# hermanjakobsen/robotic-ultrasound-imaging

Measured on AMD Instinct MI355X. Metric: env-steps/sec (whole node) at 4096 envs/GPU, random-action rollout, higher is better.
Workload: dtype f32

## Files before the change

### robotic-ultrasound-imaging_amd/csrc/usim_contact.h

```cpp
#pragma once

#define EB(off) lds[TB_WORDS + eb * GE_STRIDE + (off)]

DI float row_ror8(float x) { return __int_as_float(__builtin_amdgcn_update_dpp(0, __float_as_int(x), 0x128, 0xf, 0xf, true)); }
template <int D> DI float row_shr(float x) { return __int_as_float(__builtin_amdgcn_update_dpp(0, __float_as_int(x), 0x110 + D, 0xf, 0xf, true)); }

template <int G>
DI float group_allsum(float x) {
    if constexpr (G == 16) x += row_ror8(x);
    x += __int_as_float(__builtin_amdgcn_update_dpp(0, __float_as_int(x), 0x141, 0xf, 0xf, true));
    x += __int_as_float(__builtin_amdgcn_update_dpp(0, __float_as_int(x), 0xB1, 0xf, 0xf, true));
    x += __int_as_float(__builtin_amdgcn_update_dpp(0, __float_as_int(x), 0x4E, 0xf, 0xf, true));
    return x;
}

typedef float v2f __attribute__((ext_vector_type(2)));
struct b2 { bool x, y; };
template <class T> struct LaneVec;
template <> struct LaneVec<float> {
    typedef bool mask;
    static DI float splat(float a) { return a; }
    static DI float fma(float a, float b, float c) { return fmaf(a, b, c); }
    static DI float rcp(float a) { return rcp_(a); }
    static DI float rsq(float a) { return rsq_(a); }
    static DI float max(float a, float b) { return fmaxf(a, b); }
    static DI float min(float a, float b) { return fminf(a, b); }
    static DI bool gt(float a, float b) { return a > b; }
    static DI bool lt(float a, float b) { return a < b; }
    static DI bool both(bool a, bool b) { return bool(int(a) & int(b)); }
    static DI float sel(bool c, float a, float b) { return c ? a : b; }
    static DI float hsum(float a) { return a; }
    static DI float nsum(float a) { return -a; }
};
template <> struct LaneVec<v2f> {
    typedef b2 mask;
    static DI v2f splat(float a) { return (v2f)(a); }
    static DI v2f fma(v2f a, v2f b, v2f c) { return __builtin_elementwise_fma(a, b, c); }
    static DI v2f rcp(v2f a) { v2f r; r.x = rcp_(a.x); r.y = rcp_(a.y); return r; }
    static DI v2f rsq(v2f a) { v2f r; r.x = rsq_(a.x); r.y = rsq_(a.y); return r; }
    static DI v2f max(v2f a, v2f b) { v2f r; r.x = fmaxf(a.x, b.x); r.y = fmaxf(a.y, b.y); return r; }
    static DI v2f min(v2f a, v2f b) { v2f r; r.x = fminf(a.x, b.x); r.y = fminf(a.y, b.y); return r; }
    static DI b2 gt(v2f a, v2f b) { return b2{a.x > b.x, a.y > b.y}; }
    static DI b2 lt(v2f a, v2f b) { return b2{a.x < b.x, a.y < b.y}; }
    static DI b2 both(b2 a, b2 b) { return b2{bool(int(a.x) & int(b.x)), bool(int(a.y) & int(b.y))}; }
    static DI v2f sel(b2 c, v2f a, v2f b) { v2f r; r.x = c.x ? a.x : b.x; r.y = c.y ? a.y : b.y; return r; }
    static DI float hsum(v2f a) { return a.x + a.y; }
    static DI float nsum(v2f a) { return -a.x - a.y; }
};

template <class T>
DI typename LaneVec<T>::mask cone_local(const T b00, const T b01, const T b02, const T b11, const T b12, const T b22, T r0, T r1, T r2,
                                        const T f0, const T f1, const T f2, const T mu, T& lam, T& h0, T& h1, T& h2) {
    typedef LaneVec<T> V;
    const T Bf0 = V::fma(b02, f2, V::fma(b01, f1, b00 * f0)), Bf1 = V::fma(b12, f2, V::fma(b11, f1, b01 * f0)), Bf2 = V::fma(b22, f2, V::fma(b12, f1, b02 * f0));
    const T vr = V::fma(f2, r2, V::fma(f1, r1, f0 * r0)), vBv = V::fma(f2, Bf2, V::fma(f1, Bf1, f0 * Bf0));
    const T x = V::sel(V::gt(f0, V::splat(1e-10f)), V::max(-vr * V::rcp(vBv), V::splat(-1.f)), V::splat(0.f));
    r0 = V::fma(x, Bf0, r0); r1 = V::fma(x, Bf1, r1); r2 = V::fma(x, Bf2, r2);
    T n0 = V::fma(x, f0, f0), n1 = V::fma(x, f1, f1), n2 = V::fma(x, f2, f2);
    const T rt2 = V::fma(r1, r1, r2 * r2);
    const T irt = V::rsq(V::max(rt2, V::splat(1e-30f))), rtn = rt2 * irt;
    const T sl = V::sel(V::both(V::gt(rt2, V::splat(0.f)), V::lt(r0, mu * rtn)), -mu * irt, V::splat(0.f));
    const T u1 = sl * r1, u2 = sl * r2;
    const T Bu0 = V::fma(b02, u2, V::fma(b01, u1, b00)), Bu1 = V::fma(b12, u2, V::fma(b11, u1, b01)), Bu2 = V::fma(b22, u2, V::fma(b12, u1, b02));
    const T ur = V::fma(u2, r2, V::fma(u1, r1, r0)), uBu = V::fma(u2, Bu2, V::fma(u1, Bu1, Bu0));
    const T x2 = V::max(-ur * V::rcp(uBu), V::splat(0.f));
    n0 += x2; n1 = V::fma(x2, u1, n1); n2 = V::fma(x2, u2, n2);
    r1 = V::fma(x2, Bu1, r1); r2 = V::fma(x2, Bu2, r2);
    const T lim = mu * n0;
    const typename V::mask haslim = V::gt(lim, V::splat(1e-7f));
    const T q1 = r1 - V::fma(b12, n2, b11 * n1), q2 = r2 - V::fma(b22, n2, b12 * n1);
    T m11 = b11 + lam, m22 = b22 + lam, det = V::fma(m11, m22, -(b12 * b12));
    T a1 = V::fma(m22, q1, -(b12 * q2)), a2 = V::fma(m11, q2, -(b12 * q1));
    {
        const T aa = V::fma(a1, a1, a2 * a2);
        const T aAa = V::fma(m11 * a2, a2, V::fma(m22 * a1, a1, -2.f * b12 * a1 * a2));
        const T an = aa * V::rsq(V::max(aa, V::splat(1e-30f)));
        lam = V::max(V::fma(V::fma(-det, lim, an) * aa, V::rcp(V::max(lim * aAa, V::splat(1e-30f))), lam), V::splat(0.f));
    }
    m11 = b11 + lam; m22 = b22 + lam; det = V::fma(m11, m22, -(b12 * b12));
    a1 = V::fma(m22, q1, -(b12 * q2)); a2 = V::fma(m11, q2, -(b12 * q1));
    const T aa = V::fma(a1, a1, a2 * a2);
    const T sc = -V::min(lim * V::rsq(aa), V::rcp(det));
    h0 = n0; h1 = V::sel(haslim, a1 * sc, V::splat(0.f)); h2 = V::sel(haslim, a2 * sc, V::splat(0.f));
    return haslim;
}

DI void contact_row_geometry(const float* lds, const int eb, const int cl, const bool own, const DevModel& M, const DevCfg& C, const int nc, const int* cel, const float vz,
                             float (&w)[3][6], float (&g)[3], float (&Rd)[3], float (&Km)[MAXC], float (&vrel0)[3], float& ae0, float& kdist) {
#pragma unroll
    for (int c = 0; c < MAXC; ++c) Km[c] = 0.f;
#pragma unroll
    for (int d = 0; d < 3; ++d) {
        g[d] = 0.f; Rd[d] = 0.f; vrel0[d] = 0.f;
#pragma unroll
        for (int a = 0; a < 6; ++a) w[d][a] = 0.f;
    }
    ae0 = 0.f; kdist = 0.f;
    if (own) {
        const int b = GE_CG + cl * CG_WORDS;
        f3 nn = mk(EB(b + 0), EB(b + 1), EB(b + 2)), rr = mk(EB(b + 3), EB(b + 4), EB(b + 5));
        const int e = __float_as_int(EB(b + 6));
        const float dist = EB(b + 7);
        const float aa = -rcp_(1.f + nn.z), bb = nn.x * nn.y * aa;
        f3 t1 = mk(1.f + nn.x * nn.x * aa, bb, -nn.x);
        f3 t2 = mk(bb, 1.f + nn.y * nn.y * aa, -nn.y);
        f3 ax = mk(lds[TB_AXIS + 3 * e], lds[TB_AXIS + 3 * e + 1], lds[TB_AXIS + 3 * e + 2]);
        const float sde = EB(GE_SD + e);
        float xx = fminf(-dist * (1.0f / SI_WIDTH), 1.f);
        float yy = (xx < 0.5f) ? 2.f * xx * xx : 1.f - 2.f * (1.f - xx) * (1.f - xx);
        float dimp = SI_D0 + yy * (SI_DMAX - SI_D0);
        float kk = dimp * (1.0f / (SI_DMAX * SI_DMAX * SR_TC * SR_TC));
        float Rn = (1.f - dimp) * rcp_(dimp) * M.invw;
#pragma unroll
        for (int c = 0; c < MAXC; ++c) { const float t = lds[TB_LINV + e * LROW + cel[c]] * (1.0f / ELEM_MASS); Km[c] = (c < nc) ? t : 0.f; }
        ae0 = EB(GE_A + e);
        kdist = kk * dist;
#pragma unroll
        for (int d = 0; d < 3; ++d) {
            f3 dir = (d == 0) ? nn : (d == 1 ? t1 : t2);
            f3 rx = cross(rr, dir);
            w[d][0] = dir.x; w[d][1] = dir.y; w[d][2] = dir.z; w[d][3] = rx.x; w[d][4] = rx.y; w[d][5] = rx.z;
            g[d] = -dot(dir, ax);
            vrel0[d] = g[d] * sde - dir.z * vz;
            Rd[d] = (d == 0) ? Rn * C.rn_scale : Rn * (1.0f / IMPRATIO);
        }
    }
}
DI void contact_row_residual(const bool own, const float* Li, const float* alpha, const float* vs, const float (&w)[3][6], const float (&g)[3], const float (&vrel0)[3],
                             const float ae0, const float kdist, float (&Liw)[3][6], float (&cres)[3]) {
#pragma unroll
    for (int d = 0; d < 3; ++d) {
        cres[d] = 0.f;
#pragma unroll
        for (int a = 0; a < 6; ++a) Liw[d][a] = 0.f;
    }
    if (own) {
        const float bcon = 2.0f / (SI_DMAX * SR_TC);
#pragma unroll
        for (int d = 0; d < 3; ++d) {
// ... 87 lines not shown
        pub[4] = make_float4(Liw[2][4], Liw[2][5], g[0], g[1]); pub[5] = make_float4(g[2], 0.f, 0.f, 0.f);
    }
    group_sync();
}
DI void load_record(const float* lds, const int eb, const int k, float4 (&rk)[6]) {
    const float4* src = reinterpret_cast<const float4*>(&EB(k * 24));
#pragma unroll
    for (int v = 0; v < 6; ++v) rk[v] = src[v];
}
DI void delassus_block(const float (&w)[3][6], const float (&g)[3], const float (&Lk)[3][6], const float (&gk)[3], float (&Bj)[3][3]) {
#pragma unroll
    for (int dd = 0; dd < 3; ++dd) {
#pragma unroll
        for (int d = 0; d < 3; ++d) {
            float r1 = fmaf(w[d][4], Lk[dd][4], fmaf(w[d][2], Lk[dd][2], w[d][0] * Lk[dd][0]));
            float r2 = fmaf(w[d][5], Lk[dd][5], fmaf(w[d][3], Lk[dd][3], w[d][1] * Lk[dd][1]));
            Bj[d][dd] = fmaf(g[d], gk[dd], r1 + r2);
        }
    }
}
struct Sym3 { float b00, b01, b02, b11, b12, b22; };
template <bool CLONE, int NB>
DI void delassus_blocks(const float* lds, const int eb, const int gl, const int cl, const int ncr, const float (&w)[3][6], const float (&g)[3], const float (&Rd)[3],
                        const float (&Km)[MAXC], float (&B)[NB][3][3], Sym3& bd) {
    const bool upper = CLONE && gl >= 8 && ncr > 4;
    const int k0 = upper ? 4 : 0;
    bd = Sym3{0.f, 0.f, 0.f, 0.f, 0.f, 0.f};
    float4 rk[6];
    load_record(lds, eb, k0, rk);
#pragma unroll
    for (int j = 0; j < NB; ++j) {
        if (j < ncr) {
            float Kmj = Km[j];
            if constexpr (CLONE) Kmj = upper ? Km[4 + j] : Km[j];
            const float Lk[3][6] = {{rk[0].x, rk[0].y, rk[0].z, rk[0].w, rk[1].x, rk[1].y}, {rk[1].z, rk[1].w, rk[2].x, rk[2].y, rk[2].z, rk[2].w},
                                    {rk[3].x, rk[3].y, rk[3].z, rk[3].w, rk[4].x, rk[4].y}};
            const float gk[3] = {rk[4].z * Kmj, rk[4].w * Kmj, rk[5].x * Kmj};
            if (j + 1 < NB) load_record(lds, eb, k0 + j + 1, rk);
            delassus_block(w, g, Lk, gk, B[j]);
            const bool me = (cl - k0) == j;
            bd.b00 = me ? B[j][0][0] : bd.b00; bd.b01 = me ? B[j][0][1] : bd.b01; bd.b02 = me ? B[j][0][2] : bd.b02;
            bd.b11 = me ? B[j][1][1] : bd.b11; bd.b12 = me ? B[j][1][2] : bd.b12; bd.b22 = me ? B[j][2][2] : bd.b22;
        }
    }
    if constexpr (CLONE) {
        if (ncr > 4) {
            bd.b00 += row_ror8(bd.b00); bd.b01 += row_ror8(bd.b01); bd.b02 += row_ror8(bd.b02);
            bd.b11 += row_ror8(bd.b11); bd.b12 += row_ror8(bd.b12); bd.b22 += row_ror8(bd.b22);
        }
    }
    bd.b00 += Rd[0]; bd.b11 += Rd[1]; bd.b22 += Rd[2];
}

template <int G, bool CLONE, int NCM, int NB>
DI void delassus_product(const float (&B)[NB][3][3], const float D0, const float D1, const float D2, float& q0, float& q1, float& q2) {
    q0 = 0.f; q1 = 0.f; q2 = 0.f;
    if constexpr (NCM <= 4) {
#pragma unroll
        for (int k = 0; k < NCM; ++k) {
            const float e0 = group_bcast<G>(D0, k), e1 = group_bcast<G>(D1, k), e2 = group_bcast<G>(D2, k);
            q0 = fmaf(B[k][0][2], e2, fmaf(B[k][0][1], e1, fmaf(B[k][0][0], e0, q0)));
            q1 = fmaf(B[k][1][2], e2, fmaf(B[k][1][1], e1, fmaf(B[k][1][0], e0, q1)));
            q2 = fmaf(B[k][2][2], e2, fmaf(B[k][2][1], e1, fmaf(B[k][2][0], e0, q2)));
        }
    } else if constexpr (CLONE) {
#pragma unroll
        for (int j = 0; j < 4; ++j) {
            const float e0 = half_bcast(D0, j), e1 = half_bcast(D1, j), e2 = half_bcast(D2, j);
            q0 = fmaf(B[j][0][2], e2, fmaf(B[j][0][1], e1, fmaf(B[j][0][0], e0, q0)));
            q1 = fmaf(B[j][1][2], e2, fmaf(B[j][1][1], e1, fmaf(B[j][1][0], e0, q1)));
            q2 = fmaf(B[j][2][2], e2, fmaf(B[j][2][1], e1, fmaf(B[j][2][0], e0, q2)));
        }
        q0 += row_ror8(q0); q1 += row_ror8(q1); q2 += row_ror8(q2);
    } else {
        float h0 = 0.f, h1 = 0.f, h2 = 0.f;
#pragma unroll
        for (int k = 0; k < NCM; ++k) {
            const float e0 = group_bcast<G>(D0, k), e1 = group_bcast<G>(D1, k), e2 = group_bcast<G>(D2, k);
            float& a0 = (k < 4) ? q0 : h0; float& a1 = (k < 4) ? q1 : h1; float& a2 = (k < 4) ? q2 : h2;
            a0 = fmaf(B[k][0][2], e2, fmaf(B[k][0][1], e1, fmaf(B[k][0][0], e0, a0)));
            a1 = fmaf(B[k][1][2], e2, fmaf(B[k][1][1], e1, fmaf(B[k][1][0], e0, a1)));
            a2 = fmaf(B[k][2][2], e2, fmaf(B[k][2][1], e1, fmaf(B[k][2][0], e0, a2)));
        }
        q0 += h0; q1 += h1; q2 += h2;
    }
}

template <bool CLONE> using ContactLane = typename std::conditional<CLONE, float, v2f>::type;

template <int G, bool CLONE, bool WARM, int NCM, int NB>
DI void jacobi_iterations(const int iters, const float (&B)[NB][3][3], const Sym3& bd, const float (&Rd)[3], const typename LaneVec<ContactLane<CLONE>>::mask ownv,
                          const ContactLane<CLONE> muv, ContactLane<CLONE> (&fv)[3], ContactLane<CLONE>& lamv, float (&cres)[3]) {
    typedef ContactLane<CLONE> VT;
    typedef LaneVec<VT> V;
    const VT vb00 = V::splat(bd.b00), vb01 = V::splat(bd.b01), vb02 = V::splat(bd.b02), vb11 = V::splat(bd.b11), vb12 = V::splat(bd.b12), vb22 = V::splat(bd.b22);
    const VT vR0 = V::splat(Rd[0]), vR1 = V::splat(Rd[1]), vR2 = V::splat(Rd[2]);
    if constexpr (WARM) {
        float D0 = V::hsum(fv[0]), D1 = V::hsum(fv[1]), D2 = V::hsum(fv[2]);
        if constexpr (CLONE) { D0 += row_ror8(D0); D1 += row_ror8(D1); D2 += row_ror8(D2); }
        float q0, q1, q2;
        delassus_product<G, CLONE, NCM>(B, D0, D1, D2, q0, q1, q2);
        cres[0] += q0; cres[1] += q1; cres[2] += q2;
    }
    for (int it = 0; it < iters; ++it) {
        VT dv[3];
        float num, D0, D1, D2;
        {
            const VT r0 = V::fma(vR0, fv[0], V::splat(cres[0])), r1 = V::fma(vR1, fv[1], V::splat(cres[1])), r2 = V::fma(vR2, fv[2], V::splat(cres[2]));
            VT h0, h1, h2, lam = lamv;
            const typename V::mask haslim = cone_local<VT>(vb00, vb01, vb02, vb11, vb12, vb22, r0, r1, r2, fv[0], fv[1], fv[2], muv, lam, h0, h1, h2);
            lamv = V::sel(V::both(ownv, haslim), lam, lamv);
            dv[0] = V::sel(ownv, h0 - fv[0], V::splat(0.f)); dv[1] = V::sel(ownv, h1 - fv[1], V::splat(0.f)); dv[2] = V::sel(ownv, h2 - fv[2], V::splat(0.f));
            const VT e0 = dv[0], e1 = dv[1], e2 = dv[2];
            const VT Be0 = V::fma(vb02, e2, V::fma(vb01, e1, vb00 * e0)), Be1 = V::fma(vb12, e2, V::fma(vb11, e1, vb01 * e0)), Be2 = V::fma(vb22, e2, V::fma(vb12, e1, vb02 * e0));
            num = V::nsum(V::fma(e2, Be2, V::fma(e1, Be1, e0 * Be0)));
            D0 = V::hsum(dv[0]); D1 = V::hsum(dv[1]); D2 = V::hsum(dv[2]);
        }
        if constexpr (CLONE) { D0 += row_ror8(D0); D1 += row_ror8(D1); D2 += row_ror8(D2); }
        float q0, q1, q2;
        delassus_product<G, CLONE, NCM>(B, D0, D1, D2, q0, q1, q2);
        float den = V::hsum(V::fma(dv[2], V::fma(vR2, dv[2], V::splat(q2)), V::fma(dv[1], V::fma(vR1, dv[1], V::splat(q1)), dv[0] * V::fma(vR0, dv[0], V::splat(q0)))));
        num = group_allsum<G>(num); den = group_allsum<G>(den);
        const float t = (den > 0.f) ? fminf(-num * rcp_(den), 1.f) : 0.f;
        fv[0] = V::fma(V::splat(t), dv[0], fv[0]); fv[1] = V::fma(V::splat(t), dv[1], fv[1]); fv[2] = V::fma(V::splat(t), dv[2], fv[2]);
        cres[0] = fmaf(t, q0, cres[0]); cres[1] = fmaf(t, q1, cres[1]); cres[2] = fmaf(t, q2, cres[2]);
    }
}

template <int G, bool CLONE>
DI void contact_wrench(const int gl, const float (&w)[3][6], const float (&g)[3], const ContactLane<CLONE> (&fv)[3], float* W, float* gf) {
    float f[3];
#pragma unroll
    for (int d = 0; d < 3; ++d) {
        if constexpr (CLONE) f[d] = fv[d] + row_ror8(fv[d]);
        else f[d] = LaneVec<v2f>::hsum(fv[d]);
    }
    const float Fw[6] = {w[0][0] * f[0] + w[1][0] * f[1] + w[2][0] * f[2], w[0][1] * f[0] + w[1][1] * f[1] + w[2][1] * f[2],
                         w[0][2] * f[0] + w[1][2] * f[1] + w[2][2] * f[2], w[0][3] * f[0] + w[1][3] * f[1] + w[2][3] * f[2],
                         w[0][4] * f[0] + w[1][4] * f[1] + w[2][4] * f[2], w[0][5] * f[0] + w[1][5] * f[1] + w[2][5] * f[2]};
    const float gfo = (g[0] * f[0] + g[1] * f[1] + g[2] * f[2]) * (1.0f / ELEM_MASS);
    auto shr_add = [&](float v, auto Dc) {
        constexpr int D = decltype(Dc)::value;
        float t = row_shr<D>(v);
        if constexpr (G == 8) t = (gl < D) ? 0.f : t;
        return v + t;
    };
#pragma unroll
    for (int a = 0; a < 6; ++a) {
        float v = (gl < MAXC) ? Fw[a] : 0.f;
        v = shr_add(v, std::integral_constant<int, 1>{});
        v = shr_add(v, std::integral_constant<int, 2>{});
        v = shr_add(v, std::integral_constant<int, 4>{});
        W[a] += group_bcast<G>(v, 7);
    }
#pragma unroll
    for (int k = 0; k < MAXC; ++k) gf[k] = group_bcast<G>(gfo, k);
}

template <int G, bool PRE, class WR>
DI void contact_solve(float* lds, const int eb, const int gl, const DevModel& M, const DevCfg& C, const int nc, const int ncmax, const int* cel,
                      const float* Li, const float* alpha, const float* vs, const float mu, const float vz, const ContactRows& P, float* W, float* gf,
                      unsigned long long* dbg, WR& wr) {
    constexpr bool WARM = !std::is_same<WR, NoWarm>::value;
    constexpr bool CLONE = (G == 16) && !PRE;
    constexpr int NB = CLONE ? 4 : MAXC;
    typedef ContactLane<CLONE> VT;
    typedef LaneVec<VT> V;
    const int cl = CLONE ? (gl & 7) : gl;
    const bool own = cl < nc;
    const bool pairB = C.pair != 0;
    const float muB = fmaxf(C.probe_fric2, C.elem_fric);
    typename V::mask ownv; VT muv;
    if constexpr (CLONE) { ownv = own && (gl < 8 || pairB); muv = (gl < 8) ? mu : muB; }
    else { ownv = b2{own, own && pairB}; muv.x = mu; muv.y = muB; }

    USIM_CSTAMP(dbg, 0);
    float w[3][6], g[3], Rd[3], Km[MAXC], vrel0[3], ae0, kdist, Liw[3][6], cres[3];
    if constexpr (PRE) {
#pragma unroll
        for (int c = 0; c < MAXC; ++c) Km[c] = P.Km[c];
#pragma unroll
        for (int d = 0; d < 3; ++d) {
            g[d] = P.g[d]; Rd[d] = P.Rd[d]; vrel0[d] = P.vrel0[d];
#pragma unroll
            for (int a = 0; a < 6; ++a) w[d][a] = P.w[d][a];
        }
        ae0 = P.ae0; kdist = P.kdist;
    } else contact_row_geometry(lds, eb, cl, own, M, C, nc, cel, vz, w, g, Rd, Km, vrel0, ae0, kdist);
    contact_row_residual(own, Li, alpha, vs, w, g, vrel0, ae0, kdist, Liw, cres);
    USIM_STAMP(dbg, 9);
    USIM_CSTAMP(dbg, 1);
    float B[NB][3][3];
    Sym3 bd;
    delassus_publish(lds, eb, gl, Liw, g);
    delassus_blocks<CLONE>(lds, eb, gl, cl, ncmax, w, g, Rd, Km, B, bd);
    USIM_CSTAMP(dbg, 2);
    VT fv[3] = {V::splat(0.f), V::splat(0.f), V::splat(0.f)}, lamv = V::splat(0.f);
    int myel = -1;
    warm_match(lds, eb, gl, cl, own, ownv, wr, myel, fv, lamv);
    auto iterations = [&](auto NCM) { jacobi_iterations<G, CLONE, WARM, decltype(NCM)::value>(C.pgs_iters, B, bd, Rd, ownv, muv, fv, lamv, cres); };
    switch (ncmax) {
        case 1: iterations(std::integral_constant<int, 1>{}); break;
        case 2: iterations(std::integral_constant<int, 2>{}); break;
        case 3: iterations(std::integral_constant<int, 3>{}); break;
        case 4: iterations(std::integral_constant<int, 4>{}); break;
        case 5: iterations(std::integral_constant<int, 5>{}); break;
        case 6: iterations(std::integral_constant<int, 6>{}); break;
        case 7: iterations(std::integral_constant<int, 7>{}); break;
        default: iterations(std::integral_constant<int, 8>{}); break;
    }
    warm_keep(wr, myel, fv, lamv);
    USIM_STAMP(dbg, 10);
    USIM_CSTAMP(dbg, 3);
    contact_wrench<G, CLONE>(gl, w, g, fv, W, gf);
    USIM_CSTAMP(dbg, 4);
}

#undef EB
```

### robotic-ultrasound-imaging_amd/csrc/usim_kernels.hip

```cpp
#include <hip/hip_runtime.h>
#include <stdint.h>
#include <type_traits>
#include "usim_device.h"
#include "usim_devmath.h"

namespace usim {

constexpr int LROW = 100;
constexpr int TB_LINV = 0;
constexpr int TB_POS = N_TOP * LROW;
constexpr int TB_AXIS = TB_POS + 300;
constexpr int TB_SHELL = TB_AXIS + 300;
constexpr int TB_WORDS = TB_SHELL + 100;
constexpr int TB_ARM = TB_WORDS;
constexpr int TB_TOTAL = TB_ARM + A16_LANES * AT_STRIDE;

constexpr int GE_X = 0;
constexpr int GE_S = 100;
constexpr int GE_SD = 200;
constexpr int GE_A = 300;
constexpr int GE_U = 300;
constexpr int GE_U_WORDS = 144;
constexpr int CG_WORDS = 8;
constexpr int GE_CG = 400;
constexpr int GE_WS = 464;
constexpr int MAXCAND = 16;
constexpr int GE_STRIDE = 548;
static_assert(GE_WS + MAXC * 8 <= GE_STRIDE && GE_CG + (MAXCAND + 1) * CG_WORDS <= GE_STRIDE && GE_U + GE_U_WORDS <= GE_STRIDE, "per-environment LDS block overflow");
static_assert((LAT_NA + 2) * (LAT_NC + 2) <= GE_U_WORDS && LAT_NA * LAT_NC == N_TOP, "padded lattice grid");

constexpr int SOFT16_LDS_WORDS = TB_WORDS + 16 * GE_STRIDE;

DI void group_sync() {
    __builtin_amdgcn_fence(__ATOMIC_ACQ_REL, "workgroup");
    __builtin_amdgcn_wave_barrier();
}

#define USIM_BCAST_CASE(K)                                                                               \
    case K:                                                                                              \
        if (G == 16) iv = __builtin_amdgcn_mov_dpp(iv, 0x150 + K, 0xf, 0xf, false);                      \
        else if (G == 8) {                                                                               \
            int t = __builtin_amdgcn_mov_dpp(iv, 0x150 + K, 0xf, 0x3, false);               \
            iv = __builtin_amdgcn_update_dpp(t, iv, 0x150 + 8 + K, 0xf, 0xc, false);               \
        }                                                                                                \
        break;
template <int G>
DI float group_bcast(float v, int k) {
    int iv = __float_as_int(v);
    switch (k) {
        USIM_BCAST_CASE(0) USIM_BCAST_CASE(1) USIM_BCAST_CASE(2) USIM_BCAST_CASE(3)
        USIM_BCAST_CASE(4) USIM_BCAST_CASE(5) USIM_BCAST_CASE(6) USIM_BCAST_CASE(7)
        default: break;
    }
    return __int_as_float(iv);
}
#undef USIM_BCAST_CASE
DI float half_bcast(float v, int J) {
    const int iv = __float_as_int(v);
    int r = iv;
    switch (J) {
        case 0: { const int t = __builtin_amdgcn_mov_dpp(iv, 0x150 + 0, 0xf, 0x3, false); r = __builtin_amdgcn_update_dpp(t, iv, 0x150 + 4, 0xf, 0xc, false); } break;
        case 1: { const int t = __builtin_amdgcn_mov_dpp(iv, 0x150 + 1, 0xf, 0x3, false); r = __builtin_amdgcn_update_dpp(t, iv, 0x150 + 5, 0xf, 0xc, false); } break;
        case 2: { const int t = __builtin_amdgcn_mov_dpp(iv, 0x150 + 2, 0xf, 0x3, false); r = __builtin_amdgcn_update_dpp(t, iv, 0x150 + 6, 0xf, 0xc, false); } break;
        case 3: { const int t = __builtin_amdgcn_mov_dpp(iv, 0x150 + 3, 0xf, 0x3, false); r = __builtin_amdgcn_update_dpp(t, iv, 0x150 + 7, 0xf, 0xc, false); } break;
        default: break;
    }
    return __int_as_float(r);
}

#if !defined(USIM_TSTAMP) && !defined(USIM_TSTAMP_NOWAIT)
#define USIM_STAMP(dbg, k) do { } while (0)
#elif defined(USIM_TSTAMP_NOWAIT)
#define USIM_STAMP(dbg, k) do { if ((dbg) && blockIdx.x == 0 && threadIdx.x == 0) (dbg)[k] = __builtin_readcyclecounter(); } while (0)
#else
#define USIM_STAMP(dbg, k) do { if ((dbg) && blockIdx.x == 0 && threadIdx.x == 0) { __builtin_amdgcn_s_waitcnt(0); (dbg)[k] = __builtin_readcyclecounter(); } } while (0)
#endif

#if !defined(USIM_TSTAMP) && !defined(USIM_TSTAMP_NOWAIT)
#define USIM_CSTAMP(dbg, k) do { } while (0)
#else
#define USIM_CSTAMP(dbg, k) do { if ((dbg) && blockIdx.x == 0 && threadIdx.x == 256) (dbg)[40 + (k)] = __builtin_readcyclecounter(); } while (0)
#endif

DI void torso_motion(const DevCfg& C, int tsim, float& dz, float& vz, float& az) {
    dz = -C.drop; vz = 0.f; az = 0.f;
    if (C.torso_drop) {
        float tt = (float)tsim * C.dt, zf = -0.5f * GRAV * tt * tt;
        if (zf > -C.drop) { dz = zf; vz = -GRAV * tt; az = -GRAV; }
    }
}

DI float probe_sdf(const DevCfg& C, const f3 p, f3& g) {
    const float py = C.probe_tip - p.z - C.probe_r, e = fmaxf(fabsf(p.x) - C.probe_hl, 0.f), el = fmaxf(fabsf(p.y) - C.probe_hw, 0.f);
    const float px2 = fmaf(el, el, e * e);
    const bool pxok = px2 > 1e-18f;
    const float ipx = pxok ? rsq_(px2) : 0.f, px = px2 * ipx;
    const float kk = fmaf(py, C.probe_ca, -(px * C.probe_cb));
    const bool low = kk < 0.f, flank = !low && !(kk > C.probe_cah);
    const float qy = py - C.probe_h;
    const float lc2 = fmaf(qy, qy, px2), ll2 = fmaf(py, py, px2);
    const bool okc = lc2 > 1e-18f, okl = ll2 > 1e-18f;
    const float ilc = okc ? rsq_(lc2) : 0.f, ill = okl ? rsq_(ll2) : 0.f;
    const float cx = px * ilc, cy = qy * ilc;
    float d = low ? ll2 * ill - C.probe_r : lc2 * ilc - C.probe_r2;
    float gx = low ? px * ill : cx, gy = low ? (okl ? py * ill : -1.f) : (okc ? cy : -1.f);
    if (flank) { d = fmaf(px, C.probe_ca, fmaf(py, C.probe_cb, -C.probe_r)); gx = C.probe_ca; gy = C.probe_cb; }
    const float beta = okc ? clampf((-d - C.probe_deep0) * C.probe_inv_band, 0.f, 1.f) : 0.f;
    const float bx = fmaf(beta, cx - gx, gx), by = fmaf(beta, cy - gy, gy);
    const float rn = beta > 0.f ? rsq_(fmaf(bx, bx, by * by)) : 1.f;
    gx = bx * rn; gy = by * rn;
    const float gxi = gx * ipx;
    g = mk(copysignf(gxi * e, p.x), pxok ? copysignf(gxi * el, p.y) : gx, -gy);
    return d;
}

template <int G>
DI void collide_elem(const float* lds, float* recs, const bool valid, const int e, const int gl, const int gbase, const DevModel& M, const DevCfg& C, const float se, const float dz,
// ... 221 lines not shown
```

### robotic-ultrasound-imaging_amd/csrc/usim_step16.h

```cpp
#pragma once
#include <type_traits>

namespace usim {

template <int N, class F>
DI void static_for(F&& f) {
    if constexpr (N > 0) { static_for<N - 1>(f); f(std::integral_constant<int, N - 1>{}); }
}

template <int CTRL>
DI float dpp0(float v) { return __int_as_float(__builtin_amdgcn_update_dpp(0, __float_as_int(v), CTRL, 0xf, 0xf, true)); }
template <int G> DI int glane() { return (int)(threadIdx.x & (G - 1)); }
template <int G, int K> DI float rbc(float v) {
    if constexpr (G == 16) return dpp0<0x150 + K>(v);
    else {
        const int iv = __float_as_int(v);
        const int t = __builtin_amdgcn_update_dpp(iv, iv, 0x150 + K, 0xf, 0x3, false);
        return __int_as_float(__builtin_amdgcn_update_dpp(t, iv, 0x150 + 8 + K, 0xf, 0xc, false));
    }
}
template <int G, int D> DI float rshr0(float v) {
    const float t = dpp0<0x110 + D>(v);
    if constexpr (G == 16) return t; else return (glane<G>() < D) ? 0.f : t;
}
// ... 350 lines not shown
        int nq = __float_as_int(mb[MB_POSE + 10]);
#pragma unroll
        for (int i = arm_cull_rounds<G>(); i < NE; ++i) {
            const int eraw = i * G + gl, e = eraw < N_TOP ? eraw : N_TOP - 1;
            const bool cand = (eraw < N_TOP) && collide_cull(lds, e, M, C, s_pre[i], dz, xs, sxc, sz);
            const unsigned gm = (unsigned)(__ballot(cand) >> gbase) & GMASK;
            mb[MB_Q + (cand ? nq + __popc(gm & ((1u << gl) - 1u)) : 99)] = __int_as_float(e);
            nq += __popc(gm);
        }
        group_sync();
        int nc = 0;
        collide_queue<G>(lds, mb + MB_Q, nq, &EB(GE_CG), gl, gbase, M, C, &EB(GE_S), dz, xs, sxc, sy, sz, nc);
        constexpr bool EARLY = G == 8;
        ContactRows P;
        int nc_early = nc, overflow_early = 0, ncmax_early = 0, cel_early[MAXC];
        if constexpr (EARLY) {
            contact_overflow<G>(lds, eb, gl, gbase, nc_early);
            if (nc_early > MAXC) { overflow_early = 1; nc_early = MAXC; }
            group_sync();
#pragma unroll
            for (int k = MAXC; k >= 1; --k) if (ncmax_early == 0 && __any(nc_early >= k)) ncmax_early = k;
#pragma unroll
            for (int k = 0; k < MAXC; ++k) cel_early[k] = (k < nc_early) ? __float_as_int(EB(GE_CG + k * CG_WORDS + 6)) : 0;
            if (ncmax_early > 0) contact_rows<G>(lds, eb, gl, M, C, nc_early, cel_early, vz, P);
        }
        RSTAMP(3);
        USIM_BAR();
        RSTAMP(4);
        if constexpr (!EARLY) contact_overflow<G>(lds, eb, gl, gbase, nc);
        int overflow = 0;
        if (nc > MAXC) { overflow = 1; nc = MAXC; }
        if constexpr (!EARLY) group_sync();
        XSTAMP(0);
        int ncmax = 0;
        if constexpr (EARLY) { nc = nc_early; overflow = overflow_early; ncmax = ncmax_early; }
        else {
#pragma unroll
            for (int k = MAXC; k >= 1; --k) if (ncmax == 0 && __any(nc >= k)) ncmax = k;
        }
        XSTAMP(1);
        float gf[MAXC], W[6] = {0, 0, 0, 0, 0, 0};
        int cel[MAXC];
#pragma unroll
        for (int k = 0; k < MAXC; ++k) { const int ek = __float_as_int(EB(GE_CG + k * CG_WORDS + 6)); gf[k] = 0.f; cel[k] = EARLY ? cel_early[k] : ((k < nc) ? ek : 0); }
        if (ncmax > 0) {
            float alpha[6], vs[6], Lp[21];
#pragma unroll
            for (int a = 0; a < 6; ++a) {
                alpha[a] = mb[MB_OP + 48 + a]; vs[a] = mb[MB_OP + 54 + a];
#pragma unroll
                for (int b = 0; b <= a; ++b) Lp[PK(a, b)] = mb[MB_OP + a * 8 + b];
            }
            XSTAMP(2);
            contact_solve<G, EARLY>(lds, eb, gl, M, C, nc, ncmax, cel, Lp, alpha, vs, mu, vz, P, W, gf, dbg, cy.wr);
            XSTAMP(3);
        } else warm_clear(cy.wr);
        if (gl == 0) {
            *reinterpret_cast<float4*>(&mb[MB_W]) = make_float4(W[0], W[1], W[2], W[3]);
            *reinterpret_cast<float4*>(&mb[MB_W + 4]) = make_float4(W[4], W[5], __int_as_float(nc), __int_as_float(overflow));
#pragma unroll
            for (int k = 0; k < MAXC; ++k) { const int sh = tb_shell[cel[k]]; mb[MB_W + 8 + k] = __int_as_float((k < nc) ? sh : -1); }
        }
        RSTAMP(5);
        USIM_BAR();
        RSTAMP(6);
        {
            float acc_e[NE];
#pragma unroll
            for (int i = 0; i < NE; ++i) { const int e = gl + i * G; acc_e[i] = (e < N_TOP) ? EB(GE_A + e) : 0.f; }
#pragma unroll
            for (int k = 0; k < MAXC; ++k) {
#pragma unroll
                for (int i = 0; i < NE; ++i) {
                    const int e = (gl + i * G < N_TOP) ? gl + i * G : N_TOP - 1;
                    acc_e[i] = fmaf(lds[TB_LINV + e * LROW + cel[k]], gf[k], acc_e[i]);
                }
            }
#pragma unroll
            for (int i = 0; i < NE; ++i) {
                const int e = gl + i * G;
                if (e >= N_TOP) continue;
                const float sdn = sd_pre[i] + dt * acc_e[i];
                const float sn = s_pre[i] + dt * sdn;
                if (valid) { LAT(LAT_SD + e) = sdn; LAT(LAT_S + e) = sn; }
                if constexpr (RES) { sd_pre[i] = sdn; s_pre[i] = sn; EB(GE_S + e) = sn; }
            }
            if constexpr (WARM) { if (valid) warm_store(warm_rows, gl, cy.wr); }
        }
        RSTAMP(7);
        USIM_BAR();
        RSTAMP(8);
        return;
    }
    const int comp = gl & 3;
    const bool blk = (gl & 4) != 0;
    const bool is_task = (gl < 8) && comp != 3;
    auto pick = [&](f3 v) { return comp == 0 ? v.x : (comp == 1 ? v.y : v.z); };

    bool need = false;
    int ep_t = episode;
    if constexpr (MODE == 1) {
        need = refill ? valid : (io.mask ? io.mask[ei] != 0 : true);
        if (!__any(need)) continue;
        ep_t = refill ? item_ep : episode + 1;
        if (!refill) episode = ep_t;
        const uint32_t gid = (uint32_t)(C.env_offset + ei);
        const u4 r = philox(gid, (uint32_t)ep_t, (uint32_t)(gl < 3 ? gl : 2), 0u, C.key0, C.key1);
// ... 331 lines not shown
    float W[6] = {0, 0, 0, 0, 0, 0};
    int ncon = 0, overflow = 0, con_shell[MAXC];
#pragma unroll
    for (int k = 0; k < MAXC; ++k) con_shell[k] = -1;
    if constexpr (ROLE == 1) {
        if (is_task) {
            const int arow = blk ? 3 + comp : comp;
            float* mbo = xl + MB_OP;
            *reinterpret_cast<float4*>(&mbo[arow * 8]) = make_float4(Li[0], Li[1], Li[2], Li[3]);
            mbo[arow * 8 + 4] = Li[4]; mbo[arow * 8 + 5] = Li[5];
            mbo[48 + arow] = alpha_t; mbo[54 + arow] = v6;
        }
        RSTAMP(3);
        USIM_BAR();
        RSTAMP(4);
        precompute();
        RSTAMP(5);
        USIM_BAR();
        RSTAMP(6);
        const float4 w0 = *reinterpret_cast<const float4*>(&xl[MB_W]), w1 = *reinterpret_cast<const float4*>(&xl[MB_W + 4]);
        W[0] = w0.x; W[1] = w0.y; W[2] = w0.z; W[3] = w0.w; W[4] = w1.x; W[5] = w1.y;
        ncon = __float_as_int(w1.z); overflow = __float_as_int(w1.w);
#pragma unroll
        for (int k = 0; k < MAXC; ++k) con_shell[k] = __float_as_int(xl[MB_W + 8 + k]);
    } else if constexpr (TORSO != 0) {
        const int* tb_shell = reinterpret_cast<const int*>(lds + TB_SHELL);
        float dz, vz, az;
        torso_motion(C, tphys, dz, vz, az);
        lattice_rhs<G, NE>(lds, eb, gl, M, az, kst, kdmp, MODE == 0, s_pre, sd_pre);
        USIM_STAMP(dbg, 5);
        int nc = collide_all<G, NE>(lds, eb, gl, gbase, M, C, MODE == 0, s_pre, dz, xs, sy, sz);
        lattice_solve<G>(lds, eb, gl, gbase);
        contact_overflow<G>(lds, eb, gl, gbase, nc);
        USIM_STAMP(dbg, 7);
        if (nc > MAXC) { overflow = 1; nc = MAXC; }
        ncon = nc;
        group_sync();
        int ncmax = 0;
#pragma unroll
        for (int k = MAXC; k >= 1; --k) if (ncmax == 0 && __any(nc >= k)) ncmax = k;
        float gf[MAXC];
        int cel[MAXC];
#pragma unroll
        for (int k = 0; k < MAXC; ++k) { gf[k] = 0.f; cel[k] = (k < nc) ? __float_as_int(EB(GE_CG + k * CG_WORDS + 6)) : 0; }
        if (ncmax > 0) {
            float alpha[6], vs[6], Lp[21];
            static_for<6>([&](auto Ac) {
                constexpr int a = decltype(Ac)::value;
                alpha[a] = rbc<G, TASK_LANE[a]>(alpha_t); vs[a] = rbc<G, TASK_LANE[a]>(v6);
#pragma unroll
                for (int b = 0; b <= a; ++b) Lp[PK(a, b)] = rbc<G, TASK_LANE[a]>(Li[b]);
            });
            USIM_STAMP(dbg, 8);
            if constexpr (MODE == 0) contact_solve<G, false>(lds, eb, gl, M, C, nc, ncmax, cel, Lp, alpha, vs, mu, vz, ContactRows{}, W, gf, dbg, cy.wr);
            else { NoWarm cold; contact_solve<G, false>(lds, eb, gl, M, C, nc, ncmax, cel, Lp, alpha, vs, mu, vz, ContactRows{}, W, gf, dbg, cold); }
        } else warm_clear(cy.wr);
        USIM_STAMP(dbg, 11);
        if constexpr (MODE == 1) {
            if (valid && need && !refill) {
                for (int e = gl; e < N_TOP; e += G) { LAT(LAT_S + e) = 0.f; LAT(LAT_SD + e) = 0.f; }
                if constexpr (WARM) warm_rows_clear<G>(warm_rows, gl);
            }
        } else {
            float acc_e[NE];
#pragma unroll
            for (int i = 0; i < NE; ++i) { const int e = gl + i * G; acc_e[i] = (e < N_TOP) ? EB(GE_A + e) : 0.f; }
#pragma unroll
            for (int k = 0; k < MAXC; ++k) {
                if (k < ncmax) {
#pragma unroll
                    for (int i = 0; i < NE; ++i) {
                        const int e = (gl + i * G < N_TOP) ? gl + i * G : N_TOP - 1;
                        acc_e[i] = fmaf(lds[TB_LINV + e * LROW + cel[k]], gf[k], acc_e[i]);
                    }
                }
            }
#pragma unroll
            for (int i = 0; i < NE; ++i) {
                const int e = gl + i * G;
                if (e >= N_TOP) continue;
                const float sdn = sd_pre[i] + dt * acc_e[i];
                const float sn = s_pre[i] + dt * sdn;
                if (valid) { LAT(LAT_SD + e) = sdn; LAT(LAT_S + e) = sn; }
                if constexpr (RES) { sd_pre[i] = sdn; s_pre[i] = sn; }
            }
            if constexpr (WARM) { if (valid) warm_store(warm_rows, gl, cy.wr); }
        }
#pragma unroll
        for (int k = 0; k < MAXC; ++k) con_shell[k] = (k < nc) ? tb_shell[cel[k]] : -1;
    }
    USIM_STAMP(dbg, 12);

    if constexpr (ROLE != 1) precompute();
    float tq[3];
    f3 hv;
    {
        float qacc = qs, aq_t = alpha_t;
        if (TORSO) {
#pragma unroll
            for (int a = 0; a < 6; ++a) { qacc = fmaf(Xm[a], W[a], qacc); aq_t = fmaf(Li[a], W[a], aq_t); }
        }
        float aq[6];
        static_for<6>([&](auto Ac) { constexpr int a = decltype(Ac)::value; aq[a] = rbc<G, TASK_LANE[a]>(aq_t); });
        const f3 alq = mk(aq[3], aq[4], aq[5]);
        const f3 alt = al + alq;
        const f3 a7 = ao + mk(aq[0], aq[1], aq[2]) - cross(alq, s_xso);
        const f3 ac = a7 + cross(alt, s_rc) + s_wwrc;
        const f3 N = rot_inertia(alt) + s_nw;
// ... 213 lines not shown
```

Baseline: 221.6 million.

## Add short contact-solve path with quad DPP broadcast and paired tangent rows

Adds a SHORT template path to the contact solver, used by the step16 kernel when CLONE is active. It adds a specialised per-lane cone projection that handles the two tangent rows as a v2f pair instead of a generic vector lane. It also remaps the Delassus product broadcast to quad_perm DPP (after a row_ror layout shuffle) instead of the two-instruction half broadcast. Contact counts above four are collapsed into a single MAXC instantiation to cut code size. The cost targeted is DPP and ALU instruction count in the Jacobi iterations, at the risk of extra wasted lanes and numerical differences in the reordered arithmetic.

```diff
diff --git a/robotic-ultrasound-imaging_amd/csrc/usim_contact.h b/robotic-ultrasound-imaging_amd/csrc/usim_contact.h
--- a/robotic-ultrasound-imaging_amd/csrc/usim_contact.h
+++ b/robotic-ultrasound-imaging_amd/csrc/usim_contact.h
@@ -4,6 +4,7 @@
 
 DI float row_ror8(float x) { return __int_as_float(__builtin_amdgcn_update_dpp(0, __float_as_int(x), 0x128, 0xf, 0xf, true)); }
 template <int D> DI float row_shr(float x) { return __int_as_float(__builtin_amdgcn_update_dpp(0, __float_as_int(x), 0x110 + D, 0xf, 0xf, true)); }
+DI float quad_layout(float x) { const int ix = __float_as_int(x); return __int_as_float(__builtin_amdgcn_update_dpp(ix, ix, 0x124, 0xf, 0x6, false)); }
 
 template <int G>
 DI float group_allsum(float x) {
@@ -85,6 +86,49 @@
     return haslim;
 }
 
+DI bool cone_local_rows12(const float b00, const v2f bt, const v2f bA, const v2f bB, const v2f bD, float r0, v2f rt, const float f0, const v2f ft, const float mu,
+                          float& lam, float& h0, v2f& ht) {
+    typedef LaneVec<float> S;
+    typedef LaneVec<v2f> P;
+    const float b12 = bA.y;
+    const float Bf0 = fmaf(bt.y, ft.y, fmaf(bt.x, ft.x, b00 * f0));
+    const v2f Bft = P::fma(bB, P::splat(ft.y), P::fma(bA, P::splat(ft.x), bt * f0));
+    const float vr = fmaf(ft.y, rt.y, fmaf(ft.x, rt.x, f0 * r0)), vBv = fmaf(ft.y, Bft.y, fmaf(ft.x, Bft.x, f0 * Bf0));
+    const float x = S::sel(S::gt(f0, 1e-10f), S::max(-vr * S::rcp(vBv), -1.f), 0.f);
+    r0 = fmaf(x, Bf0, r0); rt = P::fma(P::splat(x), Bft, rt);
+    float n0 = fmaf(x, f0, f0);
+    v2f nt = P::fma(P::splat(x), ft, ft);
+    const float rt2 = fmaf(rt.x, rt.x, rt.y * rt.y);
+    const float irt = S::rsq(S::max(rt2, 1e-30f)), rtn = rt2 * irt;
+    const float sl = S::sel(S::both(S::gt(rt2, 0.f), S::lt(r0, mu * rtn)), -mu * irt, 0.f);
+    const v2f u = sl * rt;
+    const float Bu0 = fmaf(bt.y, u.y, fmaf(bt.x, u.x, b00));
+    const v2f But = P::fma(bB, P::splat(u.y), P::fma(bA, P::splat(u.x), bt));
+    const float ur = fmaf(u.y, rt.y, fmaf(u.x, rt.x, r0)), uBu = fmaf(u.y, But.y, fmaf(u.x, But.x, Bu0));
+    const float x2 = S::max(-ur * S::rcp(uBu), 0.f);
+    n0 += x2; nt = P::fma(P::splat(x2), u, nt);
+    rt = P::fma(P::splat(x2), But, rt);
+    const float lim = mu * n0;
+    const bool haslim = S::gt(lim, 1e-7f);
+    const v2f qt = rt - P::fma(bB, P::splat(nt.y), bA * nt.x);
+    v2f mt = bD + lam;
+    float det = fmaf(mt.x, mt.y, -(b12 * b12));
+    v2f at = P::fma(mt.yx, qt, -(b12 * qt.yx));
+    {
+        const float aa = fmaf(at.x, at.x, at.y * at.y);
+        const v2f ma = mt.yx * at;
+        const float aAa = fmaf(ma.y, at.y, fmaf(ma.x, at.x, -2.f * b12 * at.x * at.y));
+        const float an = aa * S::rsq(S::max(aa, 1e-30f));
+        lam = S::max(fmaf(fmaf(-det, lim, an) * aa, S::rcp(S::max(lim * aAa, 1e-30f)), lam), 0.f);
+    }
+    mt = bD + lam; det = fmaf(mt.x, mt.y, -(b12 * b12));
+    at = P::fma(mt.yx, qt, -(b12 * qt.yx));
+    const float aa = fmaf(at.x, at.x, at.y * at.y);
+    const float sc = -S::min(lim * S::rsq(aa), S::rcp(det));
+    h0 = n0; ht = haslim ? at * sc : P::splat(0.f);
+    return haslim;
+}
+
 DI void contact_row_geometry(const float* lds, const int eb, const int cl, const bool own, const DevModel& M, const DevCfg& C, const int nc, const int* cel, const float vz,
                              float (&w)[3][6], float (&g)[3], float (&Rd)[3], float (&Km)[MAXC], float (&vrel0)[3], float& ae0, float& kdist) {
 #pragma unroll
@@ -278,7 +322,7 @@
     bd.b00 += Rd[0]; bd.b11 += Rd[1]; bd.b22 += Rd[2];
 }
 
-template <int G, bool CLONE, int NCM, int NB>
+template <int G, bool CLONE, bool QUAD, int NCM, int NB>
 DI void delassus_product(const float (&B)[NB][3][3], const float D0, const float D1, const float D2, float& q0, float& q1, float& q2) {
     q0 = 0.f; q1 = 0.f; q2 = 0.f;
     if constexpr (NCM <= 4) {
@@ -290,9 +334,10 @@
             q2 = fmaf(B[k][2][2], e2, fmaf(B[k][2][1], e1, fmaf(B[k][2][0], e0, q2)));
         }
     } else if constexpr (CLONE) {
+        const float Q0 = QUAD ? quad_layout(D0) : D0, Q1 = QUAD ? quad_layout(D1) : D1, Q2 = QUAD ? quad_layout(D2) : D2;
 #pragma unroll
         for (int j = 0; j < 4; ++j) {
-            const float e0 = half_bcast(D0, j), e1 = half_bcast(D1, j), e2 = half_bcast(D2, j);
+            const float e0 = QUAD ? quad_bcast(Q0, j) : half_bcast(D0, j), e1 = QUAD ? quad_bcast(Q1, j) : half_bcast(D1, j), e2 = QUAD ? quad_bcast(Q2, j) : half_bcast(D2, j);
             q0 = fmaf(B[j][0][2], e2, fmaf(B[j][0][1], e1, fmaf(B[j][0][0], e0, q0)));
             q1 = fmaf(B[j][1][2], e2, fmaf(B[j][1][1], e1, fmaf(B[j][1][0], e0, q1)));
             q2 = fmaf(B[j][2][2], e2, fmaf(B[j][2][1], e1, fmaf(B[j][2][0], e0, q2)));
@@ -314,7 +359,7 @@
 
 template <bool CLONE> using ContactLane = typename std::conditional<CLONE, float, v2f>::type;
 
-template <int G, bool CLONE, bool WARM, int NCM, int NB>
+template <int G, bool CLONE, bool WARM, bool QUAD, bool PAIR, int NCM, int NB>
 DI void jacobi_iterations(const int iters, const float (&B)[NB][3][3], const Sym3& bd, const float (&Rd)[3], const typename LaneVec<ContactLane<CLONE>>::mask ownv,
                           const ContactLane<CLONE> muv, ContactLane<CLONE> (&fv)[3], ContactLane<CLONE>& lamv, float (&cres)[3]) {
     typedef ContactLane<CLONE> VT;
@@ -325,10 +370,37 @@
         float D0 = V::hsum(fv[0]), D1 = V::hsum(fv[1]), D2 = V::hsum(fv[2]);
         if constexpr (CLONE) { D0 += row_ror8(D0); D1 += row_ror8(D1); D2 += row_ror8(D2); }
         float q0, q1, q2;
-        delassus_product<G, CLONE, NCM>(B, D0, D1, D2, q0, q1, q2);
+        delassus_product<G, CLONE, QUAD, NCM>(B, D0, D1, D2, q0, q1, q2);
         cres[0] += q0; cres[1] += q1; cres[2] += q2;
     }
-    for (int it = 0; it < iters; ++it) {
+    if constexpr (PAIR) {
+        static_assert(CLONE, "cone_local_rows12 visits one contact per lane");
+        typedef LaneVec<v2f> P;
+        const v2f bt = {bd.b01, bd.b02}, bA = {bd.b11, bd.b12}, bB = {bd.b12, bd.b22}, bD = {bd.b11, bd.b22}, vRt = {Rd[1], Rd[2]};
+        float f0 = fv[0], c0 = cres[0];
+        v2f ft = {fv[1], fv[2]}, ct = {cres[1], cres[2]};
+        for (int it = 0; it < iters; ++it) {
+            float h0, lam = lamv;
+            v2f ht;
+            const bool haslim = cone_local_rows12(bd.b00, bt, bA, bB, bD, fmaf(Rd[0], f0, c0), P::fma(vRt, ft, ct), f0, ft, muv, lam, h0, ht);
+            lamv = V::sel(V::both(ownv, haslim), lam, lamv);
+            const float e0 = V::sel(ownv, h0 - f0, 0.f);
+            const v2f et = ownv ? ht - ft : P::splat(0.f);
+            const float Be0 = fmaf(bt.y, et.y, fmaf(bt.x, et.x, bd.b00 * e0));
+            const v2f Bet = P::fma(bB, P::splat(et.y), P::fma(bA, P::splat(et.x), bt * e0));
+            float num = -fmaf(et.y, Bet.y, fmaf(et.x, Bet.x, e0 * Be0));
+            const float D0 = e0 + row_ror8(e0), D1 = et.x + row_ror8(et.x), D2 = et.y + row_ror8(et.y);
+            float q0, q1, q2;
+            delassus_product<G, CLONE, QUAD, NCM>(B, D0, D1, D2, q0, q1, q2);
+            const v2f qt = {q1, q2}, wt = P::fma(vRt, et, qt);
+            float den = fmaf(et.y, wt.y, fmaf(et.x, wt.x, e0 * fmaf(Rd[0], e0, q0)));
+            num = group_allsum<G>(num); den = group_allsum<G>(den);
+            const float t = (den > 0.f) ? fminf(-num * rcp_(den), 1.f) : 0.f;
+            f0 = fmaf(t, e0, f0); ft = P::fma(P::splat(t), et, ft);
+            c0 = fmaf(t, q0, c0); ct = P::fma(P::splat(t), qt, ct);
+        }
+        fv[0] = f0; fv[1] = ft.x; fv[2] = ft.y; cres[0] = c0; cres[1] = ct.x; cres[2] = ct.y;
+    } else for (int it = 0; it < iters; ++it) {
         VT dv[3];
         float num, D0, D1, D2;
         {
@@ -344,7 +416,7 @@
         }
         if constexpr (CLONE) { D0 += row_ror8(D0); D1 += row_ror8(D1); D2 += row_ror8(D2); }
         float q0, q1, q2;
-        delassus_product<G, CLONE, NCM>(B, D0, D1, D2, q0, q1, q2);
+        delassus_product<G, CLONE, QUAD, NCM>(B, D0, D1, D2, q0, q1, q2);
         float den = V::hsum(V::fma(dv[2], V::fma(vR2, dv[2], V::splat(q2)), V::fma(dv[1], V::fma(vR1, dv[1], V::splat(q1)), dv[0] * V::fma(vR0, dv[0], V::splat(q0)))));
         num = group_allsum<G>(num); den = group_allsum<G>(den);
         const float t = (den > 0.f) ? fminf(-num * rcp_(den), 1.f) : 0.f;
@@ -383,13 +455,16 @@
     for (int k = 0; k < MAXC; ++k) gf[k] = group_bcast<G>(gfo, k);
 }
 
-template <int G, bool PRE, class WR>
+template <int G, bool PRE, bool SHORT, class WR>
 DI void contact_solve(float* lds, const int eb, const int gl, const DevModel& M, const DevCfg& C, const int nc, const int ncmax, const int* cel,
                       const float* Li, const float* alpha, const float* vs, const float mu, const float vz, const ContactRows& P, float* W, float* gf,
                       unsigned long long* dbg, WR& wr) {
     constexpr bool WARM = !std::is_same<WR, NoWarm>::value;
     constexpr bool CLONE = (G == 16) && !PRE;
     constexpr int NB = CLONE ? 4 : MAXC;
+    constexpr bool QUAD = CLONE && SHORT;
+    constexpr bool PAIR = CLONE && SHORT;
+    constexpr bool ONE = CLONE && SHORT;
     typedef ContactLane<CLONE> VT;
     typedef LaneVec<VT> V;
     const int cl = CLONE ? (gl & 7) : gl;
@@ -424,16 +499,16 @@
     VT fv[3] = {V::splat(0.f), V::splat(0.f), V::splat(0.f)}, lamv = V::splat(0.f);
     int myel = -1;
     warm_match(lds, eb, gl, cl, own, ownv, wr, myel, fv, lamv);
-    auto iterations = [&](auto NCM) { jacobi_iterations<G, CLONE, WARM, decltype(NCM)::value>(C.pgs_iters, B, bd, Rd, ownv, muv, fv, lamv, cres); };
-    switch (ncmax) {
+    auto iterations = [&](auto NCM) { jacobi_iterations<G, CLONE, WARM, QUAD, PAIR, decltype(NCM)::value>(C.pgs_iters, B, bd, Rd, ownv, muv, fv, lamv, cres); };
+    switch ((ONE && ncmax > 4) ? MAXC : ncmax) {
         case 1: iterations(std::integral_constant<int, 1>{}); break;
         case 2: iterations(std::integral_constant<int, 2>{}); break;
         case 3: iterations(std::integral_constant<int, 3>{}); break;
         case 4: iterations(std::integral_constant<int, 4>{}); break;
-        case 5: iterations(std::integral_constant<int, 5>{}); break;
-        case 6: iterations(std::integral_constant<int, 6>{}); break;
-        case 7: iterations(std::integral_constant<int, 7>{}); break;
-        default: iterations(std::integral_constant<int, 8>{}); break;
+        case 5: if constexpr (!ONE) iterations(std::integral_constant<int, 5>{}); break;
+        case 6: if constexpr (!ONE) iterations(std::integral_constant<int, 6>{}); break;
+        case 7: if constexpr (!ONE) iterations(std::integral_constant<int, 7>{}); break;
+        default: iterations(std::integral_constant<int, MAXC>{}); break;
     }
     warm_keep(wr, myel, fv, lamv);
     USIM_STAMP(dbg, 10);
diff --git a/robotic-ultrasound-imaging_amd/csrc/usim_kernels.hip b/robotic-ultrasound-imaging_amd/csrc/usim_kernels.hip
--- a/robotic-ultrasound-imaging_amd/csrc/usim_kernels.hip
+++ b/robotic-ultrasound-imaging_amd/csrc/usim_kernels.hip
@@ -63,6 +63,18 @@
         case 1: { const int t = __builtin_amdgcn_mov_dpp(iv, 0x150 + 1, 0xf, 0x3, false); r = __builtin_amdgcn_update_dpp(t, iv, 0x150 + 5, 0xf, 0xc, false); } break;
         case 2: { const int t = __builtin_amdgcn_mov_dpp(iv, 0x150 + 2, 0xf, 0x3, false); r = __builtin_amdgcn_update_dpp(t, iv, 0x150 + 6, 0xf, 0xc, false); } break;
         case 3: { const int t = __builtin_amdgcn_mov_dpp(iv, 0x150 + 3, 0xf, 0x3, false); r = __builtin_amdgcn_update_dpp(t, iv, 0x150 + 7, 0xf, 0xc, false); } break;
+        default: break;
+    }
+    return __int_as_float(r);
+}
+DI float quad_bcast(float v, int J) {
+    const int iv = __float_as_int(v);
+    int r = iv;
+    switch (J) {
+        case 0: r = __builtin_amdgcn_mov_dpp(iv, 0x00, 0xf, 0xf, true); break;
+        case 1: r = __builtin_amdgcn_mov_dpp(iv, 0x55, 0xf, 0xf, true); break;
+        case 2: r = __builtin_amdgcn_mov_dpp(iv, 0xAA, 0xf, 0xf, true); break;
+        case 3: r = __builtin_amdgcn_mov_dpp(iv, 0xFF, 0xf, 0xf, true); break;
         default: break;
     }
     return __int_as_float(r);
diff --git a/robotic-ultrasound-imaging_amd/csrc/usim_step16.h b/robotic-ultrasound-imaging_amd/csrc/usim_step16.h
--- a/robotic-ultrasound-imaging_amd/csrc/usim_step16.h
+++ b/robotic-ultrasound-imaging_amd/csrc/usim_step16.h
@@ -426,7 +426,7 @@
                 for (int b = 0; b <= a; ++b) Lp[PK(a, b)] = mb[MB_OP + a * 8 + b];
             }
             XSTAMP(2);
-            contact_solve<G, EARLY>(lds, eb, gl, M, C, nc, ncmax, cel, Lp, alpha, vs, mu, vz, P, W, gf, dbg, cy.wr);
+            contact_solve<G, EARLY, true>(lds, eb, gl, M, C, nc, ncmax, cel, Lp, alpha, vs, mu, vz, P, W, gf, dbg, cy.wr);
             XSTAMP(3);
         } else warm_clear(cy.wr);
         if (gl == 0) {
@@ -864,8 +864,8 @@
                 for (int b = 0; b <= a; ++b) Lp[PK(a, b)] = rbc<G, TASK_LANE[a]>(Li[b]);
             });
             USIM_STAMP(dbg, 8);
-            if constexpr (MODE == 0) contact_solve<G, false>(lds, eb, gl, M, C, nc, ncmax, cel, Lp, alpha, vs, mu, vz, ContactRows{}, W, gf, dbg, cy.wr);
-            else { NoWarm cold; contact_solve<G, false>(lds, eb, gl, M, C, nc, ncmax, cel, Lp, alpha, vs, mu, vz, ContactRows{}, W, gf, dbg, cold); }
+            if constexpr (MODE == 0) contact_solve<G, false, false>(lds, eb, gl, M, C, nc, ncmax, cel, Lp, alpha, vs, mu, vz, ContactRows{}, W, gf, dbg, cy.wr);
+            else { NoWarm cold; contact_solve<G, false, false>(lds, eb, gl, M, C, nc, ncmax, cel, Lp, alpha, vs, mu, vz, ContactRows{}, W, gf, dbg, cold); }
         } else warm_clear(cy.wr);
         USIM_STAMP(dbg, 11);
         if constexpr (MODE == 1) {
```

Measured after the change: 231.8 million (median of 6 runs). 4.6% higher.
